# MihailMihov/simd-raytracer

Measured on AMD Instinct MI355X. Metric: Mrays/s (intersect invocations per second), hw09/scene5 dragon 1920x1080 1spp, higher is better.
Workload: dtype f32; 1 GPU; BASELINE configs[1]: scenes/hw09/scene5.crtscene 1920x1080 1spp max_ray_depth=5 (primary + shadow + reflection rays), kd_tree_simd_accel semantics; rays_per_frame=2726485, primary_rays=2073600, parallelism=bucket-tiles x1

## Files before the change

### simd-raytracer_amd/csrc/api.hip

```cpp
#include <hip/hip_runtime.h>

#include <algorithm>
#include <cmath>
#include <cstdio>
#include <cstdlib>
#include <cstring>
#include <mutex>
#include <new>

#include "kernels.hpp"
#include "stream.hpp"
#include "repack.hpp"
#include "occluded.hpp"
#include "build.hpp"

namespace rtk {

static thread_local std::string g_last_error;
void set_error(const std::string &msg) { g_last_error = msg; }

namespace {

int fail(int code, const std::string &msg) { set_error(msg); return code; }

int hip_fail(hipError_t e, const char *what) {
    set_error(std::string(what) + ": " + hipGetErrorString(e));
    return RTK_ERR_HIP;
}

#define RTK_HIP(call)                                        \
    do {                                                     \
        const hipError_t e_ = (call);                        \
        if (e_ != hipSuccess) return hip_fail(e_, #call);    \
    } while (0)

template <typename T>
int upload(const std::vector<T> &src, T **dst) {
    *dst = nullptr;
    const size_t bytes = (src.empty() ? 1 : src.size()) * sizeof(T);
    RTK_HIP(hipMalloc(reinterpret_cast<void **>(dst), bytes));
    if (!src.empty()) RTK_HIP(hipMemcpy(*dst, src.data(), src.size() * sizeof(T), hipMemcpyHostToDevice));
    return RTK_OK;
}

}
}

struct rtk_knobs {
    uint32_t slice_min_tris = rtk::kSliceMinTrisDefault;
    bool shadow_exit = true;
    bool skip_unlit_shadow = true;
    bool bundle_cull = true;
    bool auto_trials = true;
    bool cost_feedback = true;
    unsigned resort_every = 16;
    uint32_t light_cycles = 140000u;
    uint32_t order_floor_cycles = 20000u;
    bool batch_scalar_surv = false;
    bool stream_scalar_surv = true;
    bool repack = true;
    bool raster_tiles = true;
    int repack_skip_bits = 6;
    bool repack_full_bounds = false;
    int repack_skip_bits2 = 14;
    bool repack_dirs3 = false;
    int repack_trace = -1;
    size_t group8_below = 9000;
    int stream_node_factor = 0;
    int stream_deep_level = 99, stream_deep_mode = RTK_TRACE_AUTO;
    uint32_t auto_min_lanes = 12;
    int stream_sort_from = -1;
    bool stream_debug = false;
    bool stream_side = true;
    int stream_lanes = 4;
    int stream_slices = 0;
    int stream_batch = 0;
    int stream_mem_gb = 96;
    int stream_side_below = 2;
    bool first_frame_prior = true;
    bool fast_occluders = true;
    bool traversal_fast = false;

    static rtk_knobs from_env() {
        rtk_knobs k;
        auto geti = [](const char *name, long &out) { const char *e = std::getenv(name); if (!e || !*e) return false; out = std::atol(e); return true; };
        long v;
        if (geti("RTK_SLICE_MIN_TRIS", v) && v > 0) k.slice_min_tris = uint32_t(v);
        if (geti("RTK_SHADOW_EARLY_EXIT", v)) k.shadow_exit = v != 0;
        if (geti("RTK_SKIP_UNLIT_SHADOW", v)) k.skip_unlit_shadow = v != 0;
        if (geti("RTK_BUNDLE_CULL", v)) k.bundle_cull = v != 0;
        if (geti("RTK_AUTO_TRIALS", v)) k.auto_trials = v != 0;
        if (geti("RTK_COST_FEEDBACK", v)) k.cost_feedback = v != 0;
        if (geti("RTK_COST_RESORT_EVERY", v) && v > 0) k.resort_every = unsigned(v);
        if (geti("RTK_LIGHT_BELOW_CYCLES", v) && v >= 0) k.light_cycles = uint32_t(v);
        if (geti("RTK_ORDER_FLOOR_CYCLES", v) && v >= 0) k.order_floor_cycles = uint32_t(v);
        if (geti("RTK_REPACK", v)) k.repack = v != 0;
        if (geti("RTK_RASTER_TILES", v)) k.raster_tiles = v != 0;
        if (geti("RTK_REPACK_FULL_BOUNDS", v)) k.repack_full_bounds = v != 0;
        if (geti("RTK_REPACK_SKIP_BITS2", v) && v >= 0 && v <= 22) k.repack_skip_bits2 = int(v);
        if (geti("RTK_REPACK_DIRS3", v)) k.repack_dirs3 = v != 0;
        if (geti("RTK_REPACK_SKIP_BITS", v) && v >= 0 && v <= 14) k.repack_skip_bits = int(v);
        if (geti("RTK_STREAM_SCALAR_SURV", v)) k.stream_scalar_surv = v != 0;
        if (geti("RTK_BATCH_SCALAR_SURV", v)) k.batch_scalar_surv = v != 0;
        if (geti("RTK_REPACK_TRACE", v) && (v == RTK_TRACE_AUTO || v == RTK_TRACE_WAVE || v == RTK_TRACE_LANE)) k.repack_trace = int(v);
        if (geti("RTK_GROUP8_BELOW_BLOCKS", v) && v >= 0) k.group8_below = size_t(v);
        if (geti("RTK_STREAM_NODE_FACTOR", v) && v >= 1) k.stream_node_factor = int(v);
        if (geti("RTK_STREAM_DEEP_LEVEL", v)) k.stream_deep_level = int(v);
        if (geti("RTK_STREAM_DEEP_MODE", v)) k.stream_deep_mode = int(v);
        if (geti("RTK_AUTO_MIN_LANES", v) && v > 0 && v <= 64) k.auto_min_lanes = uint32_t(v);
        if (geti("RTK_STREAM_SORT_FROM", v)) k.stream_sort_from = int(v);
        if (geti("RTK_STREAM_DEBUG", v)) k.stream_debug = v != 0;
        if (geti("RTK_STREAM_SIDE", v)) k.stream_side = v != 0;
        if (geti("RTK_TRAVERSAL_FAST", v)) k.traversal_fast = v != 0;
        if (geti("RTK_FIRST_FRAME_PRIOR", v)) k.first_frame_prior = v != 0;
        if (geti("RTK_STREAM_SLICES", v) && (v == 0 || v == 1 || v == 2 || v == 4)) k.stream_slices = int(v);
        if (geti("RTK_STREAM_BATCH", v) && v >= 0 && v <= 4096) k.stream_batch = int(v);
        if (geti("RTK_STREAM_MEM_GB", v) && v >= 1 && v <= 256) k.stream_mem_gb = int(v);
        if (geti("RTK_FAST_OCCLUDERS", v)) k.fast_occluders = v != 0;
        if (geti("RTK_STREAM_SIDE_BELOW", v) && v >= 0) k.stream_side_below = int(v);
        if (geti("RTK_STREAM_LANES", v) && v >= 1 && v <= rtk::dev::kStreamLanes) k.stream_lanes = int(v);
// ... 1077 lines not shown
    if (rc != RTK_OK) return rc;
    *n_floats = (g.world > 1) ? size_t(g.buckets_per_rank) * g.bucket * g.bucket * 3 : size_t(g.width) * g.height * 3;
    return RTK_OK;
}

static int render_device_impl(rtk_accel *a, const rtk_render_params *p, float *d_out, hipStream_t s) {
    FrameGeom g;
    int rc = frame_geom(a, p, g);
    if (rc != RTK_OK) return rc;
    if (!d_out) return fail(RTK_ERR_INVALID, "null output buffer");
    dev::RenderArgs A;
    std::memset(&A, 0, sizeof(A));
    A.tree = tree_view(a);
    A.materials = a->d_materials; A.lights = a->d_lights;
    A.textures = a->d_textures; A.tri_uv = a->d_tri_uv; A.tex_pixels = a->d_tex_pixels;
    A.n_lights = int(a->scene.lights.size());
    A.has_refractive = a->has_refractive ? 1 : 0;
    std::memcpy(A.cam_pos, a->scene.cam_pos, sizeof(A.cam_pos));
    std::memcpy(A.cam_mat, a->scene.cam_mat, sizeof(A.cam_mat));
    std::memcpy(A.background, a->scene.background, sizeof(A.background));
    A.width = g.width; A.height = g.height;
    A.aspect = static_cast<float>(g.width) / static_cast<float>(g.height);
    const float fov_radians = static_cast<float>(p->fov_degrees * (3.14159265358979323846 / 180.0));
    A.tan_half_fov = std::tan(fov_radians / 2.0f);
    A.spp = p->spp; A.max_depth = p->max_ray_depth; A.diffuse_rays = p->diffuse_rays; A.seed = p->seed;
    A.width_f = static_cast<float>(g.width); A.height_f = static_cast<float>(g.height);
    A.spp_f = static_cast<float>(p->spp); A.gi_div_f = static_cast<float>(p->diffuse_rays + 1);
    A.sample_begin = g.sample_begin; A.sample_end = g.sample_end;
    A.shadow_bias = p->shadow_bias; A.reflection_bias = p->reflection_bias; A.refraction_bias = p->refraction_bias;
    A.bucket = g.bucket; A.tiles_x = g.tiles_x; A.tiles_y = g.tiles_y; A.n_buckets = g.n_buckets;
    A.blocks_per_bucket_side = g.blocks_side; A.buckets_per_rank = g.buckets_per_rank;
    A.rank = g.rank; A.world = g.world; A.compact = g.world > 1 ? 1 : 0; A.skew_q = g.skew_q;
    A.out = d_out; A.counters = a->d_counters;
    A.slice_min_tris = a->knobs.slice_min_tris;
    const bool forks = a->has_refractive || p->diffuse_rays > 0;
    const bool general = forks || !a->scene.textures.empty();
    A.shadow_exit = (a->knobs.shadow_exit && !a->has_refractive && p->collect_stats != 1) ? 1 : 0;
    A.skip_unlit = (a->knobs.skip_unlit_shadow && !a->has_refractive && p->collect_stats != 1) ? 1 : 0;
    A.occl_on = (a->occl_on && p->collect_stats == 0) ? 1 : 0;
    A.occl = A.tree;
    if (A.occl_on) {
        A.occl.nodes = a->d_occl_nodes; A.occl.leaves = a->d_occl_leaves; A.occl.leaves_fast = nullptr; A.occl.n_leaves = a->occl_n_leaves;
        A.occl.tris = a->d_occl_tris; A.occl.tri_ids = a->d_occl_ids;
    }
    RTK_HIP(hipMemsetAsync(a->d_counters, 0, (kCounterWords + 4) * sizeof(unsigned long long), s));
    if (g.world > 1 && g.sample_begin == 0) {
        size_t nf = size_t(g.buckets_per_rank) * g.bucket * g.bucket * 3;
        RTK_HIP(hipMemsetAsync(d_out, 0, nf * sizeof(float), s));
    }
    bool stream = p->trace_mode == RTK_TRACE_STREAM || (p->trace_mode == RTK_TRACE_AUTO && forks);
    hipEvent_t trial_start = nullptr, trial_end = nullptr;
    if (p->trace_mode == RTK_TRACE_AUTO && forks && !p->collect_stats) {
        const bool trials = a->knobs.auto_trials;
        const uint64_t tsig[3] = {(uint64_t(uint32_t(g.width)) << 32) | uint32_t(g.height), (uint64_t(uint32_t(g.rank)) << 32) | uint32_t(g.world),
                                  (uint64_t(uint32_t(p->spp)) << 32) | (uint64_t(uint32_t(p->max_ray_depth)) << 16) | uint32_t(p->diffuse_rays)};
        if (std::memcmp(tsig, a->trial_sig, sizeof(tsig)) != 0) { std::memcpy(a->trial_sig, tsig, sizeof(tsig)); a->trial_state = 0; }
        if (trials) {
            if (!a->trial_ev[0]) for (auto &e : a->trial_ev) RTK_HIP(hipEventCreate(&e));
            if (a->trial_state == 3) {
                float t_stream = 0.f, t_mega = 0.f;
                if (hipEventQuery(a->trial_ev[1]) == hipSuccess && hipEventQuery(a->trial_ev[3]) == hipSuccess &&
                    hipEventElapsedTime(&t_stream, a->trial_ev[0], a->trial_ev[1]) == hipSuccess &&
                    hipEventElapsedTime(&t_mega, a->trial_ev[2], a->trial_ev[3]) == hipSuccess)
                    a->trial_state = t_mega < t_stream ? 5 : 4;
                else (void)hipGetLastError();
            }
            switch (a->trial_state) {
// ... 264 lines not shown

static constexpr size_t kRadianceChunkRays = size_t(1) << 22;

static int radiance_check(const rtk_accel *a, const void *rays, const void *ids, size_t n, const rtk_radiance_params *p, const void *rgb) {
    if (!a || !p) return fail(RTK_ERR_INVALID, "null accel or params");
    if (p->trace_mode != RTK_TRACE_AUTO && p->trace_mode != RTK_TRACE_STREAM)
        return fail(RTK_ERR_INVALID, "trace_mode of a radiance batch must be RTK_TRACE_AUTO or RTK_TRACE_STREAM");
    if (p->max_ray_depth < 0 || p->max_ray_depth > kMaxRayDepth) return fail(RTK_ERR_INVALID, "max_ray_depth must be in [0, 16]");
    if (p->diffuse_rays < 0 || p->diffuse_rays > 32767) return fail(RTK_ERR_INVALID, "diffuse_rays must be in [0, 32767]");
    if (p->sample < 0) return fail(RTK_ERR_INVALID, "sample must be >= 0");
    if (!std::isfinite(p->shadow_bias) || !std::isfinite(p->reflection_bias) || !std::isfinite(p->refraction_bias))
        return fail(RTK_ERR_INVALID, "shadow_bias, reflection_bias and refraction_bias must be finite");
    if (n > (size_t(1) << 38)) return fail(RTK_ERR_INVALID, "too many rays for one call");
    if (n > 0 && (!rays || !rgb)) return fail(RTK_ERR_INVALID, "null ray or colour buffer");
    if (!ids && n > (size_t(1) << 32)) return fail(RTK_ERR_INVALID, "more than 2^32 rays need explicit ids");
    return RTK_OK;
}

static int radiance_device_impl(rtk_accel *a, const rtk_ray *d_rays, const uint32_t *d_ids, size_t n, const rtk_radiance_params *p,
                                float *d_rgb, hipStream_t s, uint32_t *n_chunks_out) {
    dev::RenderArgs A;
    std::memset(&A, 0, sizeof(A));
    A.tree = tree_view(a);
    A.materials = a->d_materials; A.lights = a->d_lights;
    A.textures = a->d_textures; A.tri_uv = a->d_tri_uv; A.tex_pixels = a->d_tex_pixels;
    A.n_lights = int(a->scene.lights.size());
    A.has_refractive = a->has_refractive ? 1 : 0;
    std::memcpy(A.background, a->scene.background, sizeof(A.background));
    A.spp = 1; A.sample_begin = 0; A.sample_end = 1; A.spp_f = 1.0f;
    A.max_depth = p->max_ray_depth; A.diffuse_rays = p->diffuse_rays; A.seed = p->seed;
    A.gi_div_f = static_cast<float>(p->diffuse_rays + 1);
    A.shadow_bias = p->shadow_bias; A.reflection_bias = p->reflection_bias; A.refraction_bias = p->refraction_bias;
    A.world = 1;
    A.slice_min_tris = a->knobs.slice_min_tris;
    A.shadow_exit = (a->knobs.shadow_exit && !a->has_refractive) ? 1 : 0;
    A.skip_unlit = (a->knobs.skip_unlit_shadow && !a->has_refractive) ? 1 : 0;
    A.occl_on = a->occl_on ? 1 : 0;
    A.occl = A.tree;
    if (A.occl_on) {
        A.occl.nodes = a->d_occl_nodes; A.occl.leaves = a->d_occl_leaves; A.occl.leaves_fast = nullptr; A.occl.n_leaves = a->occl_n_leaves;
        A.occl.tris = a->d_occl_tris; A.occl.tri_ids = a->d_occl_ids;
    }
    const bool forks = a->has_refractive || p->diffuse_rays > 0;
    const size_t factor = a->knobs.stream_node_factor > 0 ? size_t(a->knobs.stream_node_factor) : (forks ? 8 : 3);
    const size_t bytes_per_node = sizeof(dev::RayRec) + sizeof(dev::NodeRes) + sizeof(uint32_t) +
                                  (sizeof(dev::HitRec) + sizeof(uint32_t) + sizeof(float2) * (a->scene.lights.empty() ? 1 : a->scene.lights.size())) / 2 + 1;
    const size_t budget = size_t(a->knobs.stream_mem_gb) << 30;
    const size_t n64 = (n + 63) / 64 * 64;
    size_t chunk = n64 < kRadianceChunkRays ? n64 : kRadianceChunkRays;
    auto fits = [&](size_t c, size_t l) { return c * factor + 4096 <= 0xF0000000ull && (c * factor + 4096) * bytes_per_node * l <= budget; };
    if (!fits(chunk, 1)) while (chunk > 64 && !fits(chunk, size_t(a->knobs.stream_lanes))) chunk = (chunk / 2 + 63) / 64 * 64;
    const size_t nodes = chunk * factor + 4096;
    const size_t n_chunks = (n + chunk - 1) / chunk;
    int lanes = n_chunks < size_t(a->knobs.stream_lanes) ? int(n_chunks) : a->knobs.stream_lanes;
    while (lanes > 1 && !fits(chunk, size_t(lanes))) lanes -= 1;
    if (n_chunks_out) *n_chunks_out = uint32_t(n_chunks);
    int rc = ensure_stream_ws(a, 0, nodes, a->scene.lights.size(), false, lanes);
    if (rc != RTK_OK) return rc;
    unsigned long long *total = nullptr;
    {
        const size_t words = size_t(dev::kStreamLanes) * kCounterWords + 2;
        if (!a->d_rad_counters) RTK_HIP(hipMalloc(reinterpret_cast<void **>(&a->d_rad_counters), words * sizeof(unsigned long long)));
        total = a->d_rad_counters + size_t(dev::kStreamLanes) * kCounterWords;
    }
    if (!a->ws_done) RTK_HIP(hipEventCreateWithFlags(&a->ws_done, hipEventDisableTiming));
    if (a->ws_in_use) RTK_HIP(hipStreamWaitEvent(s, a->ws_done, 0));
    a->ws_in_use = true;
// ... 189 lines not shown
```

### simd-raytracer_amd/csrc/kernels.hip

```cpp
#include <hip/hip_runtime.h>

#include "kernels.hpp"
#include "trace.hip.hpp"
#include "common.hip.hpp"

namespace rtk {
namespace dev {

__device__ __forceinline__ void stage_nodes(const DevNode *g_nodes, uint32_t n_nodes, DevNode *lds_nodes) {
    const float4 *src = reinterpret_cast<const float4 *>(g_nodes);
    float4 *dst = reinterpret_cast<float4 *>(lds_nodes);
    for (uint32_t i = threadIdx.x; i < n_nodes * 2u; i += blockDim.x) dst[i] = src[i];
    __syncthreads();
}

__device__ __forceinline__ void flush_stats(const Stats &st, uint32_t rays, unsigned long long *counters) {
    const uint32_t r = wave_sum(rays), h = wave_sum(st.hits), nd = wave_sum(st.nodes), bp = wave_sum(st.boxpass),
                   lv = wave_sum(st.leaves), tr = wave_sum(st.tris), pk = wave_sum(st.packets16);
    if ((threadIdx.x & 63u) == 0u) {
        atomicAdd(counters + 0, (unsigned long long)r);
        atomicAdd(counters + 2, (unsigned long long)h);
        atomicAdd(counters + 3, (unsigned long long)nd);
        atomicAdd(counters + 4, (unsigned long long)bp);
        atomicAdd(counters + 5, (unsigned long long)lv);
// ... 615 lines not shown
            } else {
                const Surface s = reconstruct(A.tree, cand);
                P = ray.o + (cand.t * ray.d);
                hn = s.hit_normal; fn = s.face_normal; din = ray.d;
                hit_tri = s.tri; hit_mat = s.material;
                if (FORKS && A.tri_uv != nullptr && A.materials[hit_mat].kind == RTK_MAT_TEXTURE)
                    albedo = sample_texture(A.textures + A.materials[hit_mat].texture, A.tri_uv + hit_tri, cand.u, cand.v, A.tex_pixels);
                state = ST_SHADE;
            }
        }
        nrays_wave += (uint32_t)__popcll(__builtin_amdgcn_ballot_w64((more_rays & 1u) != 0u)) +
                      2u * (uint32_t)__popcll(__builtin_amdgcn_ballot_w64((more_rays & 2u) != 0u)) +
                      4u * (uint32_t)__popcll(__builtin_amdgcn_ballot_w64((more_rays & 4u) != 0u)) +
                      8u * (uint32_t)__popcll(__builtin_amdgcn_ballot_w64((more_rays & 8u) != 0u));
        static_assert(kBurstMaxJobs + 1u <= 15u, "a lane's rays of one iteration fit four bits");
    }

    const uint32_t lane = fresh_lane();
#ifdef RTK_DEBUG_PHASES
    const Pixel dbg_p = my_pixel();
    const uint32_t lx = dbg_p.lx, ly = dbg_p.ly, px = dbg_p.px, py = dbg_p.py;
    if (valid && writer) {
        const unsigned long long ph_now = __builtin_readcyclecounter();
        const unsigned long long ph_rt1 = __builtin_amdgcn_s_memrealtime();
        const float vals[60] = {(float)(ph_now - ph_begin), (float)sx.c_trace, (float)sx.n_trace, (float)sx.n_steps,
                                (float)sx.n_small, (float)sx.t_small, (float)sx.c_small, (float)sx.n_big, (float)sx.t_big, (float)sx.c_big,
                                (float)(ph_begin - ph_entry), (float)(ph_first_trace - ph_begin), (float)(ph_after_first - ph_first_trace),
                                (float)(ph_now - ph_after_first), (float)sx.tally.chunks, (float)sx.tally.surv, (float)sx.tally.tris,
                                (float)(ph_rt0 & 0xFFFFFFull), (float)(ph_rt1 & 0xFFFFFFull), (float)blockIdx.x,
                                (float)ph_wait, ph_tr[0], ph_tr[1], ph_tr[2], ph_tr[3], ph_tr[4], ph_tr[5],
                                ph_kind[0], ph_kind[1], ph_kind[2], ph_kind[3], ph_kind[4], ph_kind[5], (float)sx.c_bund, (float)sx.c_list, ph_own[0],
                                (float)sx.tally.stg.n, (float)sx.tally.stg.w1, (float)sx.tally.stg.l1, (float)sx.tally.stg.w2, (float)sx.tally.stg.l2,
                                (float)sx.tally.stg.w3, (float)sx.tally.stg.l3, (float)sx.tally.stg.l4,
                                ph_job[1][0], ph_job[1][1], ph_job[1][2], ph_job[1][3], ph_job[1][4], ph_job[1][5], ph_job[1][6], ph_job[1][7],
                                ph_job[2][0], ph_job[2][1], ph_job[2][2], ph_job[2][3], ph_job[2][4], ph_job[2][5], ph_job[2][6], ph_job[2][7]};
        float v = 0.f;
        for (int i = 0; i < 60; ++i) v = (lane == (uint32_t)i) ? vals[i] : v;
        float *o = A.out + A.out_index(local_bucket, lx, ly, px, py) * 3;
        o[0] = v; o[1] = 0.f; o[2] = 0.f;
    }
#endif
    if (A.cost_out != nullptr && lane == 0u && gwave < A.n_units) {
        const unsigned long long dt = (__builtin_readcyclecounter() - cost_t0) >> (light ? 5 : 4);
        A.cost_out[gwave] = dt > 0xFFFFFFFFull ? 0xFFFFFFFFu : (uint32_t)dt;
    }
    {
        const unsigned long long dt = __builtin_amdgcn_s_memrealtime() - real_t0;
        if (lane == 0u && dt >= kCriticalMinTicks) atomicMax(A.counters + kCriticalWord + (gwave % (uint32_t)kRayCounterShards), dt);
    }
    if (SLICES > 1 && !light) group_post_exit(group_sh);
    const uint32_t total = nrays_wave;
    if (STATS && writer) flush_stats(st, 0u, A.counters);
    if (lane == 0u && writer) atomicAdd(A.counters + 8 + (gwave % (uint32_t)kRayCounterShards), (unsigned long long)total);
}

template <bool STATS, int SLICES>
__global__ __launch_bounds__(64 * SLICES, 8) void k_primary(RenderArgs A) {
    __shared__ GroupStorage<(SLICES > 1 ? SLICES : 1)> group_st;
    GroupShared *const group_sh = group_st.get();
    const uint32_t slice = (uint32_t)__builtin_amdgcn_readfirstlane((int)(((threadIdx.x >> 6) + blockIdx.x) % (uint32_t)SLICES));
    if (slice != 0u) { group_helper_loop<SLICES>(A.tree, group_sh, slice); return; }
    SliceCtx sx = {group_sh, A.slice_min_tris, 0u, true, 0u, group_sh->bundles};

    const uint32_t lane = threadIdx.x & 63u;
    const uint32_t gwave = blockIdx.x;
    const uint32_t bpb = A.blocks_per_bucket_side * A.blocks_per_bucket_side;
    const uint32_t local_bucket = gwave / bpb, sub = gwave % bpb;
// ... 395 lines not shown
```

### simd-raytracer_amd/csrc/trace.hip.hpp

```cpp
#pragma once

#include <hip/hip_runtime.h>

#include <cstddef>

#include "rtk_internal.hpp"

namespace rtk {
namespace dev {

constexpr float kFltMax = 3.402823466e+38f;
constexpr uint32_t kMiss = 0xFFFFFFFFu;

struct V3 { float x, y, z; };

__device__ __forceinline__ V3 mk(float x, float y, float z) { return V3{x, y, z}; }
__device__ __forceinline__ V3 operator+(V3 a, V3 b) { return V3{a.x + b.x, a.y + b.y, a.z + b.z}; }
__device__ __forceinline__ V3 operator-(V3 a, V3 b) { return V3{a.x - b.x, a.y - b.y, a.z - b.z}; }
__device__ __forceinline__ V3 operator*(float s, V3 a) { return V3{s * a.x, s * a.y, s * a.z}; }
__device__ __forceinline__ V3 neg(V3 a) { return V3{-a.x, -a.y, -a.z}; }
__device__ __forceinline__ float dot(V3 a, V3 b) { return (a.x * b.x) + (a.y * b.y) + (a.z * b.z); }
__device__ __forceinline__ V3 cross(V3 a, V3 b) {
    return V3{a.y * b.z - a.z * b.y, a.z * b.x - a.x * b.z, a.x * b.y - a.y * b.x};
}
// ... 544 lines not shown
    const float M_un = kT * ((TS * R.D1) * E2m) + R.dD1 * E21 + 1.0e-30f;
    const float M_vn = kT * ((TS * R.D1) * E1m) + R.dD1 * E11 + 1.0e-30f;
    const float Ax = e2y * cvz - e2z * cvy, Ay = e2z * cvx - e2x * cvz, Az = e2x * cvy - e2y * cvx;
    const float c_un = s * ((R.dcx * Ax + R.dcy * Ay) + R.dcz * Az);
    const float r_un = (__builtin_fabsf(Ax) * R.rdx + __builtin_fabsf(Ay) * R.rdy) + __builtin_fabsf(Az) * R.rdz;
    const float unH = (c_un + r_un) + M_un;
    out = out | ((unH < 0.0f) & ((-unH) * rcp >= 1.0e-30f));
    const float X1x = Ax - Dx, X1y = Ay - Dy, X1z = Az - Dz;
    const float c_x1 = s * ((R.dcx * X1x + R.dcy * X1y) + R.dcz * X1z);
    const float r_x1 = (__builtin_fabsf(X1x) * R.rdx + __builtin_fabsf(X1y) * R.rdy) + __builtin_fabsf(X1z) * R.rdz;
    out = out | (((c_x1 - r_x1) - (M_un + M_det) - slack_d) > 0.0f);
    __builtin_amdgcn_sched_barrier(0);
    const float Bx = cvy * e1z - cvz * e1y, By = cvz * e1x - cvx * e1z, Bz = cvx * e1y - cvy * e1x;
    const float c_vn = s * ((R.dcx * Bx + R.dcy * By) + R.dcz * Bz);
    const float r_vn = (__builtin_fabsf(Bx) * R.rdx + __builtin_fabsf(By) * R.rdy) + __builtin_fabsf(Bz) * R.rdz;
    const float vnH = (c_vn + r_vn) + M_vn;
    out = out | ((vnH < 0.0f) & ((-vnH) * rcp >= 1.0e-30f));
    const float X2x = X1x + Bx, X2y = X1y + By, X2z = X1z + Bz;
    const float c_x2 = s * ((R.dcx * X2x + R.dcy * X2y) + R.dcz * X2z);
    const float r_x2 = (__builtin_fabsf(X2x) * R.rdx + __builtin_fabsf(X2y) * R.rdy) + __builtin_fabsf(X2z) * R.rdz;
    out = out | (((c_x2 - r_x2) - ((M_un + M_vn) + M_det) - slack_d) > 0.0f);
    return none | (out & !(pos & neg) & (dH < 1.0e30f));
}

struct __attribute__((packed, aligned(4))) F3 { float x, y, z; };
#ifdef RTK_DEBUG_PHASES
struct CullTally { uint32_t chunks, surv, tris; unsigned long long c_cull, c_surv; StageTally stg; };
#define RTK_TALLY_ARG , CullTally &tally
#define RTK_TALLY_PASS , tally
#else
#define RTK_TALLY_ARG
#define RTK_TALLY_PASS
#endif
__device__ __forceinline__ void leaf_range_bundle(const float *tris, const uint32_t first, const uint32_t lo, const uint32_t hi,
                                                  const Ray &r, const bool cull, const float eps, const bool pass,
                                                  const uint32_t cidx, const BundleSet &BS, const bool scalar_surv, const float exit_t,
                                                  Cand &best RTK_TALLY_ARG) {
    unsigned long long pass_mask = __builtin_amdgcn_ballot_w64(pass);
    const uint32_t lane = __lane_id();
    for (uint32_t base = lo; base < hi; base += 64u) {
        if (base != lo) {
            pass_mask &= ~__builtin_amdgcn_ballot_w64(best.t <= exit_t);
            if (pass_mask == 0ull) return;
        }
#ifdef RTK_DEBUG_PHASES
        const unsigned long long pc0 = __builtin_readcyclecounter();
#endif
        const uint32_t cnt = hi - base < 64u ? hi - base : 64u;
        const bool have = lane < cnt;
        const F3 *tp = reinterpret_cast<const F3 *>(tris + (size_t)(first + base + (have ? lane : 0u)) * 9);
        const F3 v0 = tp[0], e1 = tp[1], e2 = tp[2];
        bool keep = false;
        for (uint32_t k = 0; k < BS.n; ++k) {
            if (__builtin_amdgcn_ballot_w64(pass & (cidx == k)) == 0ull) continue;
            if ((bundle_flags(BS.lds, k) & BUNDLE_PENCIL) != 0u) {
                const PencilRegs R = load_pencil(BS.lds, k);
                keep = keep | !pencil_misses(R, eps, v0.x, v0.y, v0.z, e1.x, e1.y, e1.z, e2.x, e2.y, e2.z);
            } else {
                const BundleRegs R = load_bundle(BS.lds, k, false);
                keep = keep | !bundle_misses(R.b, eps, v0.x, v0.y, v0.z, e1.x, e1.y, e1.z, e2.x, e2.y, e2.z);
            }
        }
        unsigned long long surv = __builtin_amdgcn_ballot_w64(have & keep);
#ifdef RTK_DEBUG_PHASES
        tally.chunks += 1u; tally.surv += (uint32_t)__popcll(surv); tally.tris += cnt;
#endif
#ifdef RTK_DEBUG_PHASES
        const unsigned long long ps0 = __builtin_readcyclecounter();
        tally.c_cull += ps0 - pc0;
#endif
        if (scalar_surv) {
            if (surv != 0ull) {
                cptr_f32 tb = (cptr_f32)(const void *)tris + (size_t)(first + base) * 9;
                int j = __builtin_ctzll(surv);
                surv &= surv - 1ull;
                TriS cur = load_tri_uniform(tb + (size_t)j * 9);
                for (;;) {
                    const int jn = surv != 0ull ? __builtin_ctzll(surv) : j;
                    const TriS nxt = load_tri_uniform(tb + (size_t)jn * 9);
#ifdef RTK_DEBUG_PHASES
                    tri_step(cur, first + base + (uint32_t)j, r, cull, eps, pass_mask, lane, best, &tally.stg);
#else
                    tri_step(cur, first + base + (uint32_t)j, r, cull, eps, pass_mask, lane, best);
#endif
                    if (surv == 0ull) break;
                    surv &= surv - 1ull;
                    cur = nxt; j = jn;
                }
            }
        } else {
        while (surv != 0ull) {
            const int j = __builtin_ctzll(surv);
            surv &= surv - 1ull;
            TriS cur;
            cur.v0x = __int_as_float(__builtin_amdgcn_readlane(__float_as_int(v0.x), j));
            cur.v0y = __int_as_float(__builtin_amdgcn_readlane(__float_as_int(v0.y), j));
            cur.v0z = __int_as_float(__builtin_amdgcn_readlane(__float_as_int(v0.z), j));
            cur.e1x = __int_as_float(__builtin_amdgcn_readlane(__float_as_int(e1.x), j));
            cur.e1y = __int_as_float(__builtin_amdgcn_readlane(__float_as_int(e1.y), j));
            cur.e1z = __int_as_float(__builtin_amdgcn_readlane(__float_as_int(e1.z), j));
            cur.e2x = __int_as_float(__builtin_amdgcn_readlane(__float_as_int(e2.x), j));
            cur.e2y = __int_as_float(__builtin_amdgcn_readlane(__float_as_int(e2.y), j));
            cur.e2z = __int_as_float(__builtin_amdgcn_readlane(__float_as_int(e2.z), j));
#ifdef RTK_DEBUG_PHASES
            tri_step(cur, first + base + (uint32_t)j, r, cull, eps, pass_mask, lane, best, &tally.stg);
#else
            tri_step(cur, first + base + (uint32_t)j, r, cull, eps, pass_mask, lane, best);
#endif
        }
        }
#ifdef RTK_DEBUG_PHASES
        tally.c_surv += __builtin_readcyclecounter() - ps0;
#endif
    }
}

__device__ __forceinline__ void leaf_range(const TreeView &T, const uint32_t first, const uint32_t lo, const uint32_t hi,
                                           const Ray &r, const bool cull, const bool pass, const uint32_t cidx,
                                           const BundleSet &BS, const float exit_t, Cand &best RTK_TALLY_ARG) {
    if (lo >= hi) return;
    if (BS.n != 0u && hi - lo >= kBundleMinTris)
        leaf_range_bundle(reinterpret_cast<const float *>(T.tris), first, lo, hi, r, cull, T.eps, pass, cidx, BS, T.scalar_surv != 0,
                          exit_t, best RTK_TALLY_PASS);
    else
        leaf_range_wave((cptr_f32)(const void *)T.tris, first, lo, hi, r, cull, T.eps, pass, best);
}

struct GroupShared {
    float4 ray_o[64];
    float4 ray_d[64];
    float best_t[64];
    unsigned long long pass_mask, cull_mask;
    uint32_t first, count;
    uint32_t kind;
    uint32_t ray_gen;
    uint32_t n_bundles;
    uint32_t pad[3];
    float bundles[kMaxBundles * kBundleFloats];
    float4 result[][64];
};
static_assert(offsetof(GroupShared, bundles) % 16 == 0, "bundle images are read with 16-byte LDS loads");
template <int SLICES>
struct alignas(16) GroupStorage {
    unsigned char raw[sizeof(GroupShared) + (size_t)SLICES * 64 * sizeof(float4) + (size_t)SLICES * kMaxBundles * kBundleFloats * sizeof(float)];
    __device__ __forceinline__ GroupShared *get() { return reinterpret_cast<GroupShared *>(raw); }
};
template <int SLICES>
__device__ __forceinline__ float *group_private_bundles(GroupShared *sh, const uint32_t slice) {
    return reinterpret_cast<float *>(&sh->result[SLICES][0]) + slice * (uint32_t)(kMaxBundles * kBundleFloats);
}
enum : uint32_t { GROUP_LEAF = 0, GROUP_EXIT = 1, GROUP_EXTRA = 2 };
struct NoExtraService {
    __device__ __forceinline__ void operator()(GroupShared *, uint32_t) const {}
};

struct SliceCtx {
    GroupShared *sh;
    uint32_t min_tris;
    uint32_t ray_gen;
    bool rays_dirty;
    uint32_t work;
    float *bundle_lds;
    bool rebundle = true;
#ifdef RTK_DEBUG_PHASES
    unsigned long long c_small = 0, c_big = 0, c_trace = 0, c_bund = 0, c_list = 0;
    uint32_t n_steps = 0, n_small = 0, n_big = 0, t_small = 0, t_big = 0, n_trace = 0;
    CullTally tally = {0u, 0u, 0u, 0ull, 0ull, {0u, 0u, 0u, 0u, 0u, 0u, 0u, 0u}};
#endif
};
#ifdef RTK_DEBUG_PHASES
#define RTK_SX_TALLY , sx.tally
#else
#define RTK_SX_TALLY
#endif

template <int SLICES>
__device__ __forceinline__ void slice_range(const uint32_t count, const uint32_t slice, uint32_t &lo, uint32_t &hi) {
    if (count >= 64u * (uint32_t)SLICES) {
        const uint32_t nc = (count + 63u) >> 6;
        lo = ((nc * slice) / (uint32_t)SLICES) << 6;
        hi = ((nc * (slice + 1u)) / (uint32_t)SLICES) << 6;
        lo = lo < count ? lo : count;
        hi = hi < count ? hi : count;
    } else {
        const uint32_t per = (count + (uint32_t)SLICES - 1u) / (uint32_t)SLICES;
        lo = slice * per < count ? slice * per : count;
        hi = lo + per < count ? lo + per : count;
    }
}

template <int SLICES, typename Extra = NoExtraService>
__device__ __forceinline__ void group_helper_loop(const TreeView &T, GroupShared *sh, const uint32_t slice, const Extra extra = Extra()) {
    const uint32_t lane = __lane_id();
    uint32_t my_gen = 0xFFFFFFFFu;
    Ray r;
    r.o = mk(0.f, 0.f, 0.f); r.d = mk(0.f, 0.f, 0.f); r.inv = mk(0.f, 0.f, 0.f);
    uint32_t cidx = 0u;
    BundleSet BS = {sh->bundles, 0u};
#ifdef RTK_DEBUG_PHASES
    CullTally tally = {0u, 0u, 0u, 0ull, 0ull, {0u, 0u, 0u, 0u, 0u, 0u, 0u, 0u}};
#endif
    for (;;) {
        __syncthreads();
        const uint32_t kind = (uint32_t)__builtin_amdgcn_readfirstlane((int)sh->kind);
        if (kind == GROUP_EXIT) break;
        if (kind == GROUP_EXTRA) {
            extra(sh, slice);
            my_gen = 0xFFFFFFFFu;
            __syncthreads();
            continue;
        }
        const uint32_t gen = (uint32_t)__builtin_amdgcn_readfirstlane((int)sh->ray_gen);
        if (gen != my_gen) {
            const float4 o = sh->ray_o[lane], d = sh->ray_d[lane];
            r.o = mk(o.x, o.y, o.z); r.d = mk(d.x, d.y, d.z);
            cidx = __float_as_uint(o.w);
            BS.n = (uint32_t)__builtin_amdgcn_readfirstlane((int)sh->n_bundles);
            my_gen = gen;
        }
        const uint32_t first = (uint32_t)__builtin_amdgcn_readfirstlane((int)sh->first);
        const uint32_t count = (uint32_t)__builtin_amdgcn_readfirstlane((int)sh->count);
        const unsigned long long pm = sh->pass_mask, cm = sh->cull_mask;
        Cand mine;
        mine.t = sh->best_t[lane]; mine.u = 0.f; mine.v = 0.f; mine.k = kMiss;
        uint32_t lo, hi;
        slice_range<SLICES>(count, slice, lo, hi);
        leaf_range(T, first, lo, hi, r, ((cm >> lane) & 1ull) != 0ull, ((pm >> lane) & 1ull) != 0ull, cidx, BS, sh->ray_d[lane].w,
                   mine RTK_TALLY_PASS);
        sh->result[slice][lane] = make_float4(mine.t, mine.u, mine.v, __uint_as_float(mine.k));
        __syncthreads();
    }
}

__device__ __forceinline__ void group_post_exit(GroupShared *sh) {
    if (__lane_id() == 0u) sh->kind = GROUP_EXIT;
    __syncthreads();
}

template <int SLICES>
__device__ __forceinline__ void process_leaf(const TreeView &T, const uint32_t a, const uint32_t b, const Ray &r, const bool cull,
                                             const bool pass, const uint32_t cidx, const BundleSet &BS, Cand &best, SliceCtx &sx,
                                             const float exit_t) {
    if (SLICES > 1 && b >= sx.min_tris) {
        GroupShared *sh = sx.sh;
        const uint32_t lane = __lane_id();
        if (sx.rays_dirty) {
            sh->ray_o[lane] = make_float4(r.o.x, r.o.y, r.o.z, __uint_as_float(cidx));
            sh->ray_d[lane] = make_float4(r.d.x, r.d.y, r.d.z, exit_t);
            if (lane == 0u) sh->n_bundles = BS.n;
            sx.ray_gen += 1u;
            sx.rays_dirty = false;
        }
        sh->best_t[lane] = best.t;
        const unsigned long long pm = __builtin_amdgcn_ballot_w64(pass), cm = __builtin_amdgcn_ballot_w64(cull);
        if (lane == 0u) {
            sh->pass_mask = pm; sh->cull_mask = cm;
            sh->first = a; sh->count = b; sh->kind = GROUP_LEAF; sh->ray_gen = sx.ray_gen;
        }
        __syncthreads();
        uint32_t lo0, hi0;
        slice_range<SLICES>(b, 0u, lo0, hi0);
        leaf_range(T, a, lo0, hi0, r, cull, pass, cidx, BS, exit_t, best RTK_SX_TALLY);
        __syncthreads();
#pragma unroll
        for (int s = 1; s < SLICES; ++s) {
            const float4 c = sh->result[s][lane];
            if (c.x < best.t) { best.t = c.x; best.u = c.y; best.v = c.z; best.k = __float_as_uint(c.w); }
        }
    } else {
        leaf_range(T, a, 0u, b, r, cull, pass, cidx, BS, exit_t, best RTK_SX_TALLY);
    }
}

__device__ __forceinline__ bool bundle_may_hit_box(const BundleRegs &R, const float lo0, const float lo1, const float lo2,
                                                   const float hi0, const float hi1, const float hi2) {
    const Bundle &B = R.b;
    float t_min_lo = 0.0f, t_max_hi = kFltMax;
    bool miss = false;
    if ((B.flags & BUNDLE_INVX) != 0u) {
        const Iv inv = {R.ilx, R.ihx};
        const Iv a = iv_mul(Iv{lo0 - B.ohx, lo0 - B.olx}, inv), c = iv_mul(Iv{hi0 - B.ohx, hi0 - B.olx}, inv);
        t_min_lo = __builtin_fmaxf(t_min_lo, __builtin_fminf(a.lo, c.lo));
        t_max_hi = __builtin_fminf(t_max_hi, __builtin_fmaxf(a.hi, c.hi));
        miss = t_max_hi < t_min_lo;
    }
    if ((B.flags & BUNDLE_INVY) != 0u) {
        const Iv inv = {R.ily, R.ihy};
        const Iv a = iv_mul(Iv{lo1 - B.ohy, lo1 - B.oly}, inv), c = iv_mul(Iv{hi1 - B.ohy, hi1 - B.oly}, inv);
        t_min_lo = __builtin_fmaxf(t_min_lo, __builtin_fminf(a.lo, c.lo));
        t_max_hi = __builtin_fminf(t_max_hi, __builtin_fmaxf(a.hi, c.hi));
        miss = miss | (t_max_hi < t_min_lo);
    }
    if ((B.flags & BUNDLE_INVZ) != 0u) {
        const Iv inv = {R.ilz, R.ihz};
        const Iv a = iv_mul(Iv{lo2 - B.ohz, lo2 - B.olz}, inv), c = iv_mul(Iv{hi2 - B.ohz, hi2 - B.olz}, inv);
        t_min_lo = __builtin_fmaxf(t_min_lo, __builtin_fminf(a.lo, c.lo));
        t_max_hi = __builtin_fminf(t_max_hi, __builtin_fmaxf(a.hi, c.hi));
        miss = miss | (t_max_hi < t_min_lo);
    }
    return !miss;
// ... 34 lines not shown
            if ((uint32_t)k < BS.n) {
                const BundleRegs R = load_bundle(BS.lds, (uint32_t)k, true);
                cand = cand | bundle_may_hit_box(R, q0.x, q0.y, q0.z, q0.w, q1.x, q1.y);
            }
        }
        unsigned long long cm = __builtin_amdgcn_ballot_w64(have & cand);
#ifdef RTK_DEBUG_PHASES
        sx.n_steps += (uint32_t)__popcll(cm);
        sx.c_list += __builtin_readcyclecounter() - pl0;
#endif
        while (cm != 0ull) {
            const int j = __builtin_ctzll(cm);
            cm &= cm - 1ull;
            const float lo0 = __int_as_float(__builtin_amdgcn_readlane(__float_as_int(q0.x), j));
            const float lo1 = __int_as_float(__builtin_amdgcn_readlane(__float_as_int(q0.y), j));
            const float lo2 = __int_as_float(__builtin_amdgcn_readlane(__float_as_int(q0.z), j));
            const float hi0 = __int_as_float(__builtin_amdgcn_readlane(__float_as_int(q0.w), j));
            const float hi1 = __int_as_float(__builtin_amdgcn_readlane(__float_as_int(q1.x), j));
            const float hi2 = __int_as_float(__builtin_amdgcn_readlane(__float_as_int(q1.y), j));
            float t_min;
            const bool box = slab(lo0, lo1, lo2, hi0, hi1, hi2, r, t_min);
            const bool pass = live & box & !(best.t < t_min);
            if (!wave_any(pass)) continue;
            const uint32_t a = (uint32_t)__builtin_amdgcn_readlane(__float_as_int(q1.z), j);
            const uint32_t b = (uint32_t)__builtin_amdgcn_readlane(__float_as_int(q1.w), j);
            sx.work += b + 2u;
#ifdef RTK_DEBUG_PHASES
            const unsigned long long ph0 = __builtin_readcyclecounter();
#endif
            process_leaf<SLICES>(T, a, b, r, cull, pass, cidx, BS, best, sx, exit_t);
#ifdef RTK_DEBUG_PHASES
            {
                const unsigned long long ph1 = __builtin_readcyclecounter();
                if (SLICES > 1 && b >= sx.min_tris) { sx.c_big += ph1 - ph0; sx.n_big += 1u; sx.t_big += b; }
                else { sx.c_small += ph1 - ph0; sx.n_small += 1u; sx.t_small += b; }
            }
#endif
            if (best.t <= exit_t) live = false;
            const uint32_t n_live = (uint32_t)__popcll(__builtin_amdgcn_ballot_w64(live));
            if (n_live == 0u) return;
            if (sx.rebundle && n_live * 2u <= bundled && (uint32_t)__popcll(cm) >= kRebundleMinLeaves) {
#ifdef RTK_DEBUG_PHASES
                const unsigned long long pb0 = __builtin_readcyclecounter();
#endif
                BS.n = make_bundles(r, cull, live, cls, apex, sx.bundle_lds, cidx);
#ifdef RTK_DEBUG_PHASES
                sx.c_bund += __builtin_readcyclecounter() - pb0;
#endif
                bundled = n_live;
                sx.rays_dirty = true;
            }
        }
    }
}

template <bool STATS, int SLICES>
__device__ __forceinline__ uint32_t trace_wave(const TreeView &T, const Ray &r, const bool cull, const bool active,
                                               Cand &best, Stats &st, const uint32_t min_lanes, SliceCtx &sx,
                                               const float exit_t, const uint32_t cidx, const BundleSet &BS) {
    const uint32_t end = T.n_nodes;
    uint32_t next = active ? 0u : end;
    uint32_t n = 0;
    cptr_u32 nodes = (cptr_u32)(const void *)T.nodes;
    NodeS cur = load_node_uniform(nodes);
    uint32_t have = 0u;
    while (n < end) {
        if (have != n) cur = load_node_uniform(nodes + (size_t)n * 8);
// ... 2 lines not shown
        const float lo0 = cur.lo0, lo1 = cur.lo1, lo2 = cur.lo2, hi0 = cur.hi0, hi1 = cur.hi1, hi2 = cur.hi2;
        const uint32_t a = cur.a, b = cur.b;
        cur = ahead; have = n_ahead;
        const bool part = (next == n);
        const unsigned long long part_mask = __builtin_amdgcn_ballot_w64(part);
        if (part_mask == 0ull) {
            n = (b == DEV_INNER) ? a : n + 1;
            continue;
        }
        if ((uint32_t)__popcll(part_mask) < min_lanes) break;
        float t_min;
        const bool box = slab(lo0, lo1, lo2, hi0, hi1, hi2, r, t_min);
        const bool pass = part & box & !(best.t < t_min);
        if (STATS) { st.nodes += part ? 1u : 0u; st.boxpass += pass ? 1u : 0u; }
        const bool any_pass = wave_any(pass);
        sx.work += (any_pass && b != DEV_INNER) ? b + 2u : 2u;
#ifdef RTK_DEBUG_PHASES
        sx.n_steps += 1u;
#endif
        if (b == DEV_INNER) {
            if (part) next = pass ? n + 1 : a;
            n = any_pass ? n + 1 : a;
        } else {
            if (part) next = n + 1;
            if (any_pass) {
                if (STATS && pass) { st.leaves += 1; st.tris += b; st.packets16 += (b + 15u) >> 4; }
#ifdef RTK_DEBUG_PHASES
                const unsigned long long ph0 = __builtin_readcyclecounter();
#endif
                process_leaf<SLICES>(T, a, b, r, cull, pass, cidx, BS, best, sx, exit_t);
#ifdef RTK_DEBUG_PHASES
                {
                    const unsigned long long ph1 = __builtin_readcyclecounter();
                    if (SLICES > 1 && b >= sx.min_tris) { sx.c_big += ph1 - ph0; sx.n_big += 1u; sx.t_big += b; }
                    else { sx.c_small += ph1 - ph0; sx.n_small += 1u; sx.t_small += b; }
                }
#endif
                if (best.t <= exit_t) next = end;
                if (__builtin_amdgcn_ballot_w64(next < end) == 0ull) break;
            }
            n = n + 1;
        }
    }
    return next;
}

constexpr uint32_t kAutoMinLanes = 12;

__device__ __forceinline__ bool enters_root(const TreeView &T, const Ray &r, const bool active) {
    cptr_u32 nodes = (cptr_u32)(const void *)T.nodes;
    const NodeS root = load_node_uniform(nodes);
    float t_min;
    return active & slab(root.lo0, root.lo1, root.lo2, root.hi0, root.hi1, root.hi2, r, t_min);
}

template <int MODE, bool STATS, bool LDS_NODES, int SLICES = 1, bool ROOT_DONE = false>
__device__ __forceinline__ Cand trace(const TreeView &T, const DevNode *lds_nodes, const Ray &r, const bool cull,
                                      const bool active, Stats &st, SliceCtx &sx, const uint32_t auto_min = kAutoMinLanes,
                                      const float exit_t = -1.0f, const uint32_t cls = 0u, const V3 apex = V3{0.f, 0.f, 0.f}) {
    static_assert(!(ROOT_DONE && STATS), "the counting build walks every node, the root included");
    Cand best;
    best.t = kFltMax; best.u = 0.0f; best.v = 0.0f; best.k = kMiss;
    sx.rays_dirty = true;
    if (MODE == RTK_TRACE_LANE) {
        trace_lane_from<STATS, LDS_NODES>(T, lds_nodes, r, cull, active ? 0u : T.n_nodes, best, st, exit_t);
    } else if (MODE == RTK_TRACE_WAVE) {
        if (wave_any(active)) {
// ... 60 lines not shown
```

Baseline: 14150 Mrays/s.

## Deal big-leaf triangle chunks to slice waves via a shared atomic ticket

Replaces the static split of large leaves across workgroup waves with dynamic dealing. Each wave draws chunk-sized triangle ranges from an LDS atomic counter, so waves whose rays cull more triangles keep pulling work instead of waiting at the barrier. The chunk size is packed into the low bits of slice_min_tris. Merging results now breaks ties by candidate index so the output is deterministic. This adds one atomic and readfirstlane per chunk, and chunks narrower than 64 leave lanes idle per pass.

```diff
diff --git a/simd-raytracer_amd/csrc/api.hip b/simd-raytracer_amd/csrc/api.hip
--- a/simd-raytracer_amd/csrc/api.hip
+++ b/simd-raytracer_amd/csrc/api.hip
@@ -48,6 +48,8 @@
 
 struct rtk_knobs {
     uint32_t slice_min_tris = rtk::kSliceMinTrisDefault;
+    bool slice_deal = true;
+    uint32_t slice_chunk = 64;
     bool shadow_exit = true;
     bool skip_unlit_shadow = true;
     bool bundle_cull = true;
@@ -86,6 +88,8 @@
         auto geti = [](const char *name, long &out) { const char *e = std::getenv(name); if (!e || !*e) return false; out = std::atol(e); return true; };
         long v;
         if (geti("RTK_SLICE_MIN_TRIS", v) && v > 0) k.slice_min_tris = uint32_t(v);
+        if (geti("RTK_SLICE_DEAL", v)) k.slice_deal = v != 0;
+        if (geti("RTK_SLICE_CHUNK", v) && v >= 8 && v <= 64) k.slice_chunk = uint32_t(v);
         if (geti("RTK_SHADOW_EARLY_EXIT", v)) k.shadow_exit = v != 0;
         if (geti("RTK_SKIP_UNLIT_SHADOW", v)) k.skip_unlit_shadow = v != 0;
         if (geti("RTK_BUNDLE_CULL", v)) k.bundle_cull = v != 0;
@@ -1229,7 +1233,7 @@
     A.blocks_per_bucket_side = g.blocks_side; A.buckets_per_rank = g.buckets_per_rank;
     A.rank = g.rank; A.world = g.world; A.compact = g.world > 1 ? 1 : 0; A.skew_q = g.skew_q;
     A.out = d_out; A.counters = a->d_counters;
-    A.slice_min_tris = a->knobs.slice_min_tris;
+    A.slice_min_tris = dev::slice_word(a->knobs.slice_min_tris, (a->knobs.slice_deal && p->collect_stats == 0) ? a->knobs.slice_chunk : 0u);
     const bool forks = a->has_refractive || p->diffuse_rays > 0;
     const bool general = forks || !a->scene.textures.empty();
     A.shadow_exit = (a->knobs.shadow_exit && !a->has_refractive && p->collect_stats != 1) ? 1 : 0;
@@ -1560,7 +1564,7 @@
     A.gi_div_f = static_cast<float>(p->diffuse_rays + 1);
     A.shadow_bias = p->shadow_bias; A.reflection_bias = p->reflection_bias; A.refraction_bias = p->refraction_bias;
     A.world = 1;
-    A.slice_min_tris = a->knobs.slice_min_tris;
+    A.slice_min_tris = dev::slice_word(a->knobs.slice_min_tris, a->knobs.slice_deal ? a->knobs.slice_chunk : 0u);
     A.shadow_exit = (a->knobs.shadow_exit && !a->has_refractive) ? 1 : 0;
     A.skip_unlit = (a->knobs.skip_unlit_shadow && !a->has_refractive) ? 1 : 0;
     A.occl_on = a->occl_on ? 1 : 0;
diff --git a/simd-raytracer_amd/csrc/kernels.hip b/simd-raytracer_amd/csrc/kernels.hip
--- a/simd-raytracer_amd/csrc/kernels.hip
+++ b/simd-raytracer_amd/csrc/kernels.hip
@@ -671,7 +671,7 @@
                                 ph_kind[0], ph_kind[1], ph_kind[2], ph_kind[3], ph_kind[4], ph_kind[5], (float)sx.c_bund, (float)sx.c_list, ph_own[0],
                                 (float)sx.tally.stg.n, (float)sx.tally.stg.w1, (float)sx.tally.stg.l1, (float)sx.tally.stg.w2, (float)sx.tally.stg.l2,
                                 (float)sx.tally.stg.w3, (float)sx.tally.stg.l3, (float)sx.tally.stg.l4,
-                                ph_job[1][0], ph_job[1][1], ph_job[1][2], ph_job[1][3], ph_job[1][4], ph_job[1][5], ph_job[1][6], ph_job[1][7],
+                                (float)sx.c_wall, (float)sx.c_busy_max, (float)sx.c_busy_sum, (float)sx.s_max, (float)sx.s_sum, (float)sx.n_dealt, ph_job[1][6], ph_job[1][7],
                                 ph_job[2][0], ph_job[2][1], ph_job[2][2], ph_job[2][3], ph_job[2][4], ph_job[2][5], ph_job[2][6], ph_job[2][7]};
         float v = 0.f;
         for (int i = 0; i < 60; ++i) v = (lane == (uint32_t)i) ? vals[i] : v;
diff --git a/simd-raytracer_amd/csrc/trace.hip.hpp b/simd-raytracer_amd/csrc/trace.hip.hpp
--- a/simd-raytracer_amd/csrc/trace.hip.hpp
+++ b/simd-raytracer_amd/csrc/trace.hip.hpp
@@ -600,27 +600,30 @@
 #define RTK_TALLY_ARG
 #define RTK_TALLY_PASS
 #endif
+__device__ __forceinline__ uint32_t draw_pass(uint32_t *ticket, const uint32_t deal) {
+    uint32_t c = 0u;
+    if (__lane_id() == 0u) c = __hip_atomic_fetch_add(ticket, 1u, __ATOMIC_RELAXED, __HIP_MEMORY_SCOPE_WORKGROUP);
+    return (uint32_t)__builtin_amdgcn_readfirstlane((int)c) * deal;
+}
 __device__ __forceinline__ void leaf_range_bundle(const float *tris, const uint32_t first, const uint32_t lo, const uint32_t hi,
                                                   const Ray &r, const bool cull, const float eps, const bool pass,
                                                   const uint32_t cidx, const BundleSet &BS, const bool scalar_surv, const float exit_t,
-                                                  Cand &best RTK_TALLY_ARG) {
+                                                  Cand &best RTK_TALLY_ARG, uint32_t *ticket = nullptr, const uint32_t deal = 0u) {
     unsigned long long pass_mask = __builtin_amdgcn_ballot_w64(pass);
     const uint32_t lane = __lane_id();
-    for (uint32_t base = lo; base < hi; base += 64u) {
-        if (base != lo) {
-            pass_mask &= ~__builtin_amdgcn_ballot_w64(best.t <= exit_t);
-            if (pass_mask == 0ull) return;
-        }
+    uint32_t base = deal != 0u ? draw_pass(ticket, deal) : lo;
+    while (base < hi) {
 #ifdef RTK_DEBUG_PHASES
         const unsigned long long pc0 = __builtin_readcyclecounter();
 #endif
-        const uint32_t cnt = hi - base < 64u ? hi - base : 64u;
+        const uint32_t width = deal != 0u ? deal : 64u;
+        const uint32_t cnt = hi - base < width ? hi - base : width;
         const bool have = lane < cnt;
         const F3 *tp = reinterpret_cast<const F3 *>(tris + (size_t)(first + base + (have ? lane : 0u)) * 9);
         const F3 v0 = tp[0], e1 = tp[1], e2 = tp[2];
         bool keep = false;
         for (uint32_t k = 0; k < BS.n; ++k) {
-            if (__builtin_amdgcn_ballot_w64(pass & (cidx == k)) == 0ull) continue;
+            if ((__builtin_amdgcn_ballot_w64(cidx == k) & pass_mask) == 0ull) continue;
             if ((bundle_flags(BS.lds, k) & BUNDLE_PENCIL) != 0u) {
                 const PencilRegs R = load_pencil(BS.lds, k);
                 keep = keep | !pencil_misses(R, eps, v0.x, v0.y, v0.z, e1.x, e1.y, e1.z, e2.x, e2.y, e2.z);
@@ -680,16 +683,20 @@
 #ifdef RTK_DEBUG_PHASES
         tally.c_surv += __builtin_readcyclecounter() - ps0;
 #endif
+        pass_mask &= ~__builtin_amdgcn_ballot_w64(best.t <= exit_t);
+        if (pass_mask == 0ull) return;
+        base = deal != 0u ? draw_pass(ticket, deal) : base + 64u;
     }
 }
 
 __device__ __forceinline__ void leaf_range(const TreeView &T, const uint32_t first, const uint32_t lo, const uint32_t hi,
                                            const Ray &r, const bool cull, const bool pass, const uint32_t cidx,
-                                           const BundleSet &BS, const float exit_t, Cand &best RTK_TALLY_ARG) {
+                                           const BundleSet &BS, const float exit_t, Cand &best RTK_TALLY_ARG,
+                                           uint32_t *ticket = nullptr, const uint32_t deal = 0u) {
     if (lo >= hi) return;
     if (BS.n != 0u && hi - lo >= kBundleMinTris)
         leaf_range_bundle(reinterpret_cast<const float *>(T.tris), first, lo, hi, r, cull, T.eps, pass, cidx, BS, T.scalar_surv != 0,
-                          exit_t, best RTK_TALLY_PASS);
+                          exit_t, best RTK_TALLY_PASS, ticket, deal);
     else
         leaf_range_wave((cptr_f32)(const void *)T.tris, first, lo, hi, r, cull, T.eps, pass, best);
 }
@@ -704,6 +711,9 @@
     uint32_t ray_gen;
     uint32_t n_bundles;
     uint32_t pad[3];
+#ifdef RTK_DEBUG_PHASES
+    uint32_t dbg_busy[16], dbg_surv[16];
+#endif
     float bundles[kMaxBundles * kBundleFloats];
     float4 result[][64];
 };
@@ -721,6 +731,13 @@
 struct NoExtraService {
     __device__ __forceinline__ void operator()(GroupShared *, uint32_t) const {}
 };
+
+constexpr uint32_t kSliceChunkBits = 7;
+constexpr uint32_t kSliceChunkMask = (1u << kSliceChunkBits) - 1u;
+__host__ __device__ inline uint32_t slice_word(const uint32_t min_tris, const uint32_t deal_chunk) {
+    const uint32_t m = min_tris < (0xFFFFFFFFu >> kSliceChunkBits) ? min_tris : (0xFFFFFFFFu >> kSliceChunkBits);
+    return (m << kSliceChunkBits) | (deal_chunk <= 64u ? deal_chunk : 64u);
+}
 
 struct SliceCtx {
     GroupShared *sh;
@@ -734,6 +751,8 @@
     unsigned long long c_small = 0, c_big = 0, c_trace = 0, c_bund = 0, c_list = 0;
     uint32_t n_steps = 0, n_small = 0, n_big = 0, t_small = 0, t_big = 0, n_trace = 0;
     CullTally tally = {0u, 0u, 0u, 0ull, 0ull, {0u, 0u, 0u, 0u, 0u, 0u, 0u, 0u}};
+    unsigned long long c_wall = 0, c_busy_max = 0, c_busy_sum = 0;
+    uint32_t s_max = 0, s_sum = 0, n_dealt = 0;
 #endif
 };
 #ifdef RTK_DEBUG_PHASES
@@ -757,6 +776,22 @@
     }
 }
 
+template <int SLICES>
+__device__ __forceinline__ uint32_t deal_chunk_of(const SliceCtx &sx, const BundleSet &BS, const uint32_t count) {
+    const uint32_t chunk = sx.min_tris & kSliceChunkMask;
+    return (chunk != 0u && BS.n != 0u && count >= chunk * (uint32_t)SLICES) ? chunk : 0u;
+}
+
+template <int SLICES>
+__device__ __forceinline__ void slice_passes(const TreeView &T, GroupShared *sh, const uint32_t first, const uint32_t count,
+                                             const uint32_t slice, const uint32_t chunk, const Ray &r, const bool cull, const bool pass,
+                                             const uint32_t cidx, const BundleSet &BS, const float exit_t, Cand &best RTK_TALLY_ARG) {
+    uint32_t lo, hi;
+    slice_range<SLICES>(count, slice, lo, hi);
+    const bool dealt = chunk != 0u;
+    leaf_range(T, first, dealt ? 0u : lo, dealt ? count : hi, r, cull, pass, cidx, BS, exit_t, best RTK_TALLY_PASS, &sh->pad[1], chunk);
+}
+
 template <int SLICES, typename Extra = NoExtraService>
 __device__ __forceinline__ void group_helper_loop(const TreeView &T, GroupShared *sh, const uint32_t slice, const Extra extra = Extra()) {
     const uint32_t lane = __lane_id();
@@ -791,10 +826,16 @@
         const unsigned long long pm = sh->pass_mask, cm = sh->cull_mask;
         Cand mine;
         mine.t = sh->best_t[lane]; mine.u = 0.f; mine.v = 0.f; mine.k = kMiss;
-        uint32_t lo, hi;
-        slice_range<SLICES>(count, slice, lo, hi);
-        leaf_range(T, first, lo, hi, r, ((cm >> lane) & 1ull) != 0ull, ((pm >> lane) & 1ull) != 0ull, cidx, BS, sh->ray_d[lane].w,
-                   mine RTK_TALLY_PASS);
+        const uint32_t chunk = (uint32_t)__builtin_amdgcn_readfirstlane((int)sh->pad[2]);
+#ifdef RTK_DEBUG_PHASES
+        const unsigned long long hb0 = __builtin_readcyclecounter();
+        const uint32_t hs0 = tally.surv;
+#endif
+        slice_passes<SLICES>(T, sh, first, count, slice, chunk, r, ((cm >> lane) & 1ull) != 0ull, ((pm >> lane) & 1ull) != 0ull, cidx, BS,
+                             sh->ray_d[lane].w, mine RTK_TALLY_PASS);
+#ifdef RTK_DEBUG_PHASES
+        if (lane == 0u) { sh->dbg_busy[slice & 15u] = (uint32_t)(__builtin_readcyclecounter() - hb0); sh->dbg_surv[slice & 15u] = tally.surv - hs0; }
+#endif
         sh->result[slice][lane] = make_float4(mine.t, mine.u, mine.v, __uint_as_float(mine.k));
         __syncthreads();
     }
@@ -809,7 +850,7 @@
 __device__ __forceinline__ void process_leaf(const TreeView &T, const uint32_t a, const uint32_t b, const Ray &r, const bool cull,
                                              const bool pass, const uint32_t cidx, const BundleSet &BS, Cand &best, SliceCtx &sx,
                                              const float exit_t) {
-    if (SLICES > 1 && b >= sx.min_tris) {
+    if (SLICES > 1 && b >= (sx.min_tris >> kSliceChunkBits)) {
         GroupShared *sh = sx.sh;
         const uint32_t lane = __lane_id();
         if (sx.rays_dirty) {
@@ -821,19 +862,39 @@
         }
         sh->best_t[lane] = best.t;
         const unsigned long long pm = __builtin_amdgcn_ballot_w64(pass), cm = __builtin_amdgcn_ballot_w64(cull);
+        const uint32_t chunk = deal_chunk_of<SLICES>(sx, BS, b);
         if (lane == 0u) {
             sh->pass_mask = pm; sh->cull_mask = cm;
             sh->first = a; sh->count = b; sh->kind = GROUP_LEAF; sh->ray_gen = sx.ray_gen;
+            sh->pad[1] = 0u; sh->pad[2] = chunk;
         }
         __syncthreads();
-        uint32_t lo0, hi0;
-        slice_range<SLICES>(b, 0u, lo0, hi0);
-        leaf_range(T, a, lo0, hi0, r, cull, pass, cidx, BS, exit_t, best RTK_SX_TALLY);
+#ifdef RTK_DEBUG_PHASES
+        const unsigned long long ob0 = __builtin_readcyclecounter();
+        const uint32_t os0 = sx.tally.surv;
+#endif
+        slice_passes<SLICES>(T, sh, a, b, 0u, chunk, r, cull, pass, cidx, BS, exit_t, best RTK_SX_TALLY);
+#ifdef RTK_DEBUG_PHASES
+        const unsigned long long ob1 = __builtin_readcyclecounter();
+#endif
         __syncthreads();
+#ifdef RTK_DEBUG_PHASES
+        {
+            uint32_t bmax = (uint32_t)(ob1 - ob0), bsum = bmax, smax = sx.tally.surv - os0, ssum = smax;
+            for (int s = 1; s < SLICES; ++s) {
+                const uint32_t hb = (uint32_t)__builtin_amdgcn_readfirstlane((int)sh->dbg_busy[s & 15]);
+                const uint32_t hs = (uint32_t)__builtin_amdgcn_readfirstlane((int)sh->dbg_surv[s & 15]);
+                bmax = hb > bmax ? hb : bmax; bsum += hb; smax = hs > smax ? hs : smax; ssum += hs;
+            }
+            sx.c_wall += __builtin_readcyclecounter() - ob0; sx.c_busy_max += bmax; sx.c_busy_sum += bsum;
+            sx.s_max += smax; sx.s_sum += ssum; sx.n_dealt += chunk != 0u ? 1u : 0u;
+        }
+#endif
 #pragma unroll
         for (int s = 1; s < SLICES; ++s) {
             const float4 c = sh->result[s][lane];
-            if (c.x < best.t) { best.t = c.x; best.u = c.y; best.v = c.z; best.k = __float_as_uint(c.w); }
+            const uint32_t ck = __float_as_uint(c.w);
+            if ((c.x < best.t) | ((c.x == best.t) & (ck < best.k))) { best.t = c.x; best.u = c.y; best.v = c.z; best.k = ck; }
         }
     } else {
         leaf_range(T, a, 0u, b, r, cull, pass, cidx, BS, exit_t, best RTK_SX_TALLY);
@@ -934,7 +995,7 @@
 #ifdef RTK_DEBUG_PHASES
             {
                 const unsigned long long ph1 = __builtin_readcyclecounter();
-                if (SLICES > 1 && b >= sx.min_tris) { sx.c_big += ph1 - ph0; sx.n_big += 1u; sx.t_big += b; }
+                if (SLICES > 1 && b >= (sx.min_tris >> kSliceChunkBits)) { sx.c_big += ph1 - ph0; sx.n_big += 1u; sx.t_big += b; }
                 else { sx.c_small += ph1 - ph0; sx.n_small += 1u; sx.t_small += b; }
             }
 #endif
@@ -1003,7 +1064,7 @@
 #ifdef RTK_DEBUG_PHASES
                 {
                     const unsigned long long ph1 = __builtin_readcyclecounter();
-                    if (SLICES > 1 && b >= sx.min_tris) { sx.c_big += ph1 - ph0; sx.n_big += 1u; sx.t_big += b; }
+                    if (SLICES > 1 && b >= (sx.min_tris >> kSliceChunkBits)) { sx.c_big += ph1 - ph0; sx.n_big += 1u; sx.t_big += b; }
                     else { sx.c_small += ph1 - ph0; sx.n_small += 1u; sx.t_small += b; }
                 }
 #endif
```

New measurement: 14040 Mrays/s. No clear change (-0.8%).
